# VCISwang/STCD

Hardware: AMD Instinct MI355X
Metric: image-pairs/sec (256x256 bf16 SiamUnet_diff train) (higher is better)
Workload: dtype bf16; 1 GPU; SiamUnet_diff(3,2) 256x256 full training step (fwd + cross_entropy + bwd + AdamW), 16 pairs/GPU, synthetic LEVIR-CD-shaped pairs resident in HBM; global_batch=16, image=256, parallelism=dp1

## Files before the change

stcd_amd/csrc/common.h:

```cpp
#pragma once
#include <hip/hip_runtime.h>
#include <stdint.h>
#include <stdio.h>
#include <stdlib.h>
#include <string>
#include <string.h>

#include "../../include/stcd_hip.h"

namespace stcd {

typedef __bf16 bf16;

enum DType { F32 = STCD_DTYPE_F32, BF16 = STCD_DTYPE_BF16 };
inline size_t dsize(int dt) { return dt == BF16 ? 2 : 4; }

void set_error(const std::string& msg);

static inline int env_int(const char* name, int dflt) { const char* v = getenv(name); return v ? atoi(v) : dflt; }
static inline bool env_flag(const char* name, bool dflt) { const char* v = getenv(name); return v && v[0] == (dflt ? '0' : '1') ? !dflt : dflt; }

#define STCD_CHECK_AS(fn, cond, msg)                                       \
    do {                                                                   \
        if (!(cond)) {                                                     \
// ... 336 lines not shown
};
ConvDmaPlan conv_dma_plan(const stcd_conv_geom& g, const ConvMfmaPlan& p);
int launch_conv_dma(const stcd_conv_geom& g, const ConvMfmaPlan& p, const ConvDmaPlan& dp, const ConvArgs& c);

bool conv_small_ok(const stcd_conv_geom& g, const ConvMfmaPlan& p);
int conv_small_blocks(const stcd_conv_geom& g, int groups);
int launch_conv_small(const stcd_conv_geom& g, const ConvArgs& c);
bool conv_small_call_ok(const stcd_conv_geom& g, int groups, const XfSrc* xf);
bool conv_small_bwdsum_ok(const stcd_conv_geom& g);
struct WgradMfmaPlan {
    int WCI = 1, NTW = 1, gx = 1, gy = 1, gz = 1;
    int64_t slab_floats = 0;
    int wi_valid = 0;
    int gemm = 0;
    int dma = 0;
    bool ok = false;
};
WgradMfmaPlan wgrad_mfma_plan(const stcd_conv_geom& g, int kpad, int wld, bool allow_wide = false, int force_co64 = -1);
int launch_wgrad_mfma(const stcd_conv_geom& g, const WgradMfmaPlan& p, const void* in, const void* dout, float* slab,
                      int kpad, int wld, hipStream_t s);
struct WgradJob {
    stcd_conv_geom g;
    int64_t in_off, dout_off, slab_off;
    int kpad, wld;
    int dymin, dxmin, HH, HWp;
    int tiles_x, tiles_y, ntiles;
    int xrow_bytes;
    int x_bytes, y_bytes;
    int co_valid;
    unsigned in_bytes, dout_bytes;
    int gx, gy, gz;
    int start;
    int lds_bytes;
    int wi_valid;
    int dma_L, dma_nk;
    int pad_;
    int64_t xf_stat_off, xf_mask_off;
    int xf_C, xf_groups, xf_npg, pad2_;
};
WgradMfmaPlan wgrad_gemm_plan(const stcd_conv_geom& g, int kpad, int wld);
WgradMfmaPlan wgrad_dma_plan(const stcd_conv_geom& g, int kpad, int wld);
void wgrad_dma_set_split(WgradMfmaPlan& p, const stcd_conv_geom& g, int S, int kpad, int wld);
WgradJob wgrad_dma_make_job(const stcd_conv_geom& g, const WgradMfmaPlan& p, int64_t in_off, int64_t dout_off, int64_t slab_off,
                            int kpad, int wld);
int launch_wgrad_dma_group(const WgradJob* jobs_dev, int njobs, int total_blocks, const char* base, hipStream_t s);
struct WgradKernel {
    enum Kind { TILE, GEMM, DMA } kind = TILE;
    int WCI = 0, NTW = 0; bool t9 = false, xf = false;
    int W = 0;
    bool operator==(const WgradKernel& o) const { return kind == o.kind && WCI == o.WCI && NTW == o.NTW && t9 == o.t9 && xf == o.xf && W == o.W; }
};
struct WgradXf { int64_t stat_off = -1, mask_off = -1; int C = 0, groups = 1, npg = 1; };
WgradKernel wgrad_kernel_of(const WgradMfmaPlan& p, const stcd_conv_geom& g, bool xf);
bool wgrad_kernel_takes_xf(const WgradKernel& k);
void wgrad_kernel_name(const WgradKernel& k, bool grouped, char out[64]);
int wgrad_variant_slots(const WgradKernel& k, int lds_bytes);
WgradJob wgrad_job(const WgradKernel& k, const stcd_conv_geom& g, const WgradMfmaPlan& p, int64_t in_off, int64_t dout_off,
                   int64_t slab_off, int kpad, int wld, const WgradXf* xf = nullptr);
int launch_wgrad_jobs(const WgradKernel& k, const WgradJob* jobs_dev, int njobs, int total_blocks, int lds_bytes, const char* base,
                      hipStream_t s);
struct PackSpec;
struct ReduceJob {
// ... 293 lines not shown
```

stcd_amd/csrc/engine.hip:

```cpp
#include <algorithm>
#include <climits>
#include <cstdint>
#include <array>
#include <cstring>
#include <memory>
#include <vector>

#include "common.h"

namespace stcd {

static thread_local std::string g_err;
void set_error(const std::string& msg) { g_err = msg; }

enum ConvKind { K_CONV3 = 0, K_CONVT3_S1 = 1, K_UPCONV = 2, K_CONV1 = 3, K_CONVT2 = 4, K_CONV3_S2 = 5, K_CONV1_S2 = 6, K_STEM7 = 7 };

struct TRef { int64_t off = -1; int ld = 0; };
struct GRef { int64_t off = -1; int ld = 0; int64_t goff = 0; };

static inline int round8(int c) { return (c + 7) & ~7; }

struct ConvW {
    std::string name;
    int kind = 0, cin = 0, cout = 0;
// ... 232 lines not shown
    int64_t jobs_total[2] = {0, 0}, jobs_off[2] = {-1, -1};
    const void* jobs_uploaded_ws = nullptr;
    uint64_t weights_tag = 0, packed_tag = 0;
    const void* packed_ws = nullptr; const void* packed_params = nullptr; int packed_level = -1;
    TRef X0, G, finalIn, dFinalIn;
    int Hs[5] = {0}, Ws[5] = {0};
    TRef D[4], dD[4], P[4], dP[4];
    int64_t zero_begin = -1, zero_end = -1;
    int64_t final_bias_acc = -1;
    std::vector<BiasJob> bias_jobs; int64_t bias_jobs_off = -1;
    int64_t masks = -1, dwe_begin = -1, dwe_end = -1, scratch8 = -1;
    int use_mfma = 1, use_small = 1, use_wgroup = 1, use_res = 1, use_skip_fused = 1, use_act_fuse = 1, use_gemm = 1, use_skip_recompute = 1, use_bwdsum = 1, use_bwdsum_res = 0, use_tile = 1, use_halo = 0;
    int wg_side_on = 1;
    static constexpr int WG_SIDE_DIV = 4;
    static constexpr int WGROUP_ROUNDS = 1, WGROUP_MIN_TILES = 8;
    hipStream_t wg_side = nullptr; hipEvent_t wg_fork = nullptr, wg_join = nullptr; int wg_side_dev = -1;
};

}

using namespace stcd;
struct stcd_engine : stcd_engine_impl {};

namespace stcd {

static const int ENC_STAGE_CONVS[4] = {2, 2, 3, 3};
static const int ENC_C[4] = {16, 32, 64, 128};
static const int SKIP_IDX[4] = {1, 3, 6, 9};

static void add_param(stcd_engine& e, const std::string& name, std::initializer_list<int64_t> shape, int64_t* off_out) {
// ... 417 lines not shown
static void split_tile_group(const stcd_engine& e, int stage, const WgradGroup& G, const std::vector<WgradOp*>& ops) {
    int64_t W = 0;
    for (const WgradOp* op : ops) W += wgrad_ntiles(op->g) * op->plan.gy * op->plan.gz;
    int slots = wgrad_variant_slots(G.kernel, G.lds_bytes);
    if (stage == 0 && e.wg_side_on && fc_family(e)) slots = std::max(64, slots / stcd_engine_impl::WG_SIDE_DIV);
    const int64_t rounds = stcd_engine_impl::WGROUP_ROUNDS;
    const int64_t tpb = std::max<int64_t>(stcd_engine_impl::WGROUP_MIN_TILES, (W + rounds * slots - 1) / (rounds * slots));
    for (WgradOp* op : ops) {
        const int64_t slab = wgrad_slab_floats(e, *op);
        int64_t gx = std::max<int64_t>(1, (wgrad_ntiles(op->g) + tpb - 1) / tpb);
        gx = std::min<int64_t>(gx, std::max<int64_t>(1, ((int64_t)32 << 20) / (slab * 4)));
        op->plan.gx = (int)gx;
        op->plan.slab_floats = gx * slab;
    }
}
static void choose_wgroup_splits(stcd_engine& e) {
    for (int st = 0; st < 2; ++st)
        for (size_t gi = 0; gi < e.wgroups[st].size(); ++gi) {
            WgradGroup& G = e.wgroups[st][gi];
            std::vector<WgradOp*> ops;
            for (WgradOp* op : e.wgrad_ops)
                if (op->stage == st && op->group == (int)gi) ops.push_back(op);
            for (const WgradOp* op : ops)
                G.lds_bytes = std::max(G.lds_bytes, wgrad_job_of(e, G.kernel, *op, 0, 0, 0).lds_bytes);
            if (G.kernel.kind == WgradKernel::DMA) split_dma_group(e, ops);
            else if (G.kernel.kind == WgradKernel::TILE) split_tile_group(e, st, G, ops);
        }
}

static void take_wgrad_slabs(stcd_engine& e, Planner& ws) {
    for (WgradOp* op : e.wgrad_ops) {
        if (!op->plan.ok) continue;
        op->slab = ws.take(op->plan.slab_floats * 4);
        if (op->group < 0) continue;
        WgradGroup& G = e.wgroups[op->stage][op->group];
        WgradJob j = wgrad_job_of(e, G.kernel, *op, op->in_off, op->dout_off, op->slab);
        j.start = G.total_blocks;
        G.total_blocks += j.gx * j.gy * j.gz;
        G.jobs.push_back(j);
        double fl, by;
        conv_work(e, op->g, op->kreal, op->nreal, &fl, &by);
        G.flops += fl; G.bytes += by;
// ... 45 lines not shown
        const int k = op->group == last->group ? 1 : 0;
        tot[k] = append_reduce_job(part[k], tot[k], e.rjobs[1][part[0].size() + part[1].size()]);
    }
    if (part[0].empty() || part[1].empty()) return;
    e.rjobs[1] = part[0];
    e.rjobs[1].insert(e.rjobs[1].end(), part[1].begin(), part[1].end());
    e.rj_split = (int)part[0].size(); e.wg_final_group = last->group;
    e.rj_total_early = tot[0]; e.rj_total_final = tot[1];
}

static void build_wgrad_jobs(stcd_engine& e, Planner& ws) {
    for (int st = 0; st < 2; ++st) { e.rjobs[st].clear(); e.rjobs_total[st] = 0; e.wgroups[st].clear(); }
    e.rj_split = 0; e.wg_final_group = -1; e.rj_total_early = e.rj_total_final = 0;
    if (e.dt == BF16 && e.use_mfma) {
        if (e.use_wgroup) { form_wgroups(e); choose_wgroup_splits(e); }
        take_wgrad_slabs(e, ws);
        build_reduce_tables(e);
        split_reduce_final(e);
        for (int st = 0; st < 2; ++st) {
            e.rjobs_off[st] = ws.take((int64_t)e.rjobs[st].size() * sizeof(ReduceJob) + 16);
            for (WgradGroup& G : e.wgroups[st]) G.table_off = ws.take((int64_t)G.jobs.size() * sizeof(WgradJob) + 16);
        }
    }
    for (int st = 0; st < 2; ++st) e.wrun.groups[st].assign(e.wgroups[st].size(), WgradRun::Group());
}

static void build_filter_pack_jobs(stcd_engine& e, Planner& ws) {
    for (int with_dgrad = 0; with_dgrad < 2; ++with_dgrad) {
        std::vector<PackJob>& jobs = e.jobs[with_dgrad];
        jobs.clear();
// ... 38 lines not shown
                }
                push(j);
            }
        }
        e.jobs_total[with_dgrad] = cur;
        e.jobs_off[with_dgrad] = ws.take((int64_t)jobs.size() * sizeof(PackJob) + 16);
    }
}

static int configure_fcsiam(stcd_engine& e, int B, int H, int W) {
    const int64_t T = (int64_t)dsize(e.dt);
    const int ND = fc_dates(e);
    e.Hs[0] = H; e.Ws[0] = W;
    for (int s = 0; s < 4; ++s) { e.Hs[s + 1] = e.Hs[s] / 2; e.Ws[s + 1] = e.Ws[s] / 2; }
    Planner ws(e);
    auto add_drop = [&](const std::string& name, int rows, int C) {
        DropP d; d.name = name; d.rows = rows; d.C = C; d.off = e.drop_floats;
        e.drop_floats += (int64_t)rows * C;
        e.drops.push_back(d);
        return (int)e.drops.size() - 1;
    };

    e.X0 = ws.plain(ND * B, H, W, 8);
    for (int s = 0; s < 4; ++s) {
        int Cd = ENC_C[s] + (e.arch == STCD_ARCH_CONC ? 2 : 1) * ENC_C[s];
        e.D[s] = ws.plain(B, e.Hs[s], e.Ws[s], Cd);
        e.dD[s] = ws.plain(B, e.Hs[s], e.Ws[s], Cd);
        e.P[s] = ws.plain(ND * B, e.Hs[s + 1], e.Ws[s + 1], ENC_C[s]);
        e.dP[s] = ws.plain(ND * B, e.Hs[s + 1], e.Ws[s + 1], ENC_C[s]);
    }
// ... 2028 lines not shown
        else {
            launch_slice(dt, c.at(st.ddst.off), st.ddst.ld, c.at(e.g_pool_idc.off), e.g_pool_idc.ld, (int64_t)st.N * (st.h / 2) * (st.w / 2), st.C, 1, s);
            launch_maxpool3_bwd(dt, c.at<unsigned char>(e.g_pool_idx), c.at(st.ddst.off), st.ddst.ld, c.at(st.dsrc.off), st.dsrc.ld, st.N, st.h, st.w, st.C, s);
        }
    }
    if (stage_tail(c, 0, nullptr, false, finish_biases)) return 1;
    STCD_HIP(hipGetLastError());
    return 0;
}

#include "engine_cf.inl"

static void reset_plan(stcd_engine& e) {
    e.enc.clear(); e.dec.clear(); e.ups.clear();
    e.drops.clear(); e.drop_floats = 0;
    e.conv_ops.clear(); e.wgrad_ops.clear(); e.slab_floats = 0; e.wg_last_op = nullptr;
    e.ws_tensors.clear(); e.bias_jobs.clear();
    e.g_fwd.clear(); e.sn_order.clear();
    if (e.cf) cf_reset_plan(*e.cf);
}

}

extern "C" {

const char* stcd_last_error(void) { return stcd::g_err.c_str(); }
int stcd_abi_version(void) { return STCD_ABI_VERSION; }

static void engine_env_switches(stcd_engine* e) {
    e->use_mfma = !env_flag("STCD_FORCE_REF_KERNELS", false);
    e->use_small = !env_flag("STCD_NO_SMALL_KERNEL", false);
// ... 460 lines not shown
    STCD_CHECK((g->hm - 1) * g->out_stride + g->oy0 < g->ho && (g->wm - 1) * g->out_stride + g->ox0 < g->wo,
               "output positions exceed the output buffer");
    return 0;
}
static int op_dma_splits(const stcd_conv_geom& g, const WgradMfmaPlan& p) {
    const int64_t M = (int64_t)g.n * g.hi * g.wi;
    return (int)std::max<int64_t>(1, std::min<int64_t>(256 / std::max(1, p.gy * p.gz), M / 512));
}
int64_t stcd_op_scratch_bytes(const stcd_conv_geom* g) {
    if (!g) return 0;
    ConvMfmaPlan p = conv_mfma_plan(*g);
    WgradMfmaPlan w = wgrad_mfma_plan(*g, g->ci, g->co), ww = wgrad_mfma_plan(*g, g->ci, g->co, true);
    WgradMfmaPlan wg = wgrad_gemm_plan(*g, g->ci, g->co);
    WgradMfmaPlan wd = wgrad_dma_plan(*g, g->ci, g->co);
    if (wd.ok) wgrad_dma_set_split(wd, *g, op_dma_splits(*g, wd), g->ci, g->co);
    return std::max<int64_t>(p.wf_elems * 2, std::max(std::max(std::max(w.slab_floats, ww.slab_floats), wg.ok ? wg.slab_floats : 0), wd.ok ? wd.slab_floats : 0) * 4) + 1024;
}
int stcd_op_conv(int dtype, int impl, const stcd_conv_geom* g, const void* in, const float* w, const float* bias,
                 void* out, void* scratch, int64_t scratch_bytes, void* hip_stream) {
    if (check_geom(g)) return 1;
    STCD_CHECK(in && w && out, "null pointer argument");
    if (impl == 1 || impl == 2 || impl == 3 || impl == 6 || impl == 8) {
        STCD_CHECK(dtype == STCD_DTYPE_BF16, "the MFMA implementation is bf16 only");
        ConvOp op;
        op.g = *g;
        op.plan = conv_mfma_plan(*g);
        const ConvMfmaPlan& p = op.plan;
        STCD_CHECK(p.ok, "geometry not supported by the MFMA kernel");
        STCD_CHECK(scratch && scratch_bytes >= p.wf_elems * 2, "scratch too small for the fragment-order filter");
        launch_pack_frag(*g, p, w, g->ci, g->co, scratch, (hipStream_t)hip_stream);
        ConvArgs a;
// ... 112 lines not shown
}
int stcd_op_wgrad(int dtype, int impl, const stcd_conv_geom* g, const void* in, const void* dout, float* dw, void* scratch,
                  int64_t scratch_bytes, void* hip_stream) {
    if (check_geom(g)) return 1;
    STCD_CHECK(in && dout && dw, "null pointer argument");
    if (impl == 1 || impl == 4 || impl == 5) {
        STCD_CHECK(dtype == STCD_DTYPE_BF16, "the MFMA implementation is bf16 only");
        WgradMfmaPlan p = wgrad_mfma_plan(*g, g->ci, g->co, impl >= 4, impl == 5 ? 1 : 0);
        STCD_CHECK(p.ok, "geometry not supported by the MFMA kernel");
        STCD_CHECK(scratch && scratch_bytes >= p.slab_floats * 4, "scratch too small for the partial slabs");
        STCD_CHECK(launch_wgrad_mfma(*g, p, in, dout, (float*)scratch, g->ci, g->co, (hipStream_t)hip_stream) == 0, "LDS budget exceeded");
        launch_reduce_dw((const float*)scratch, p.gx, *g, g->ci, g->co, g->ci, g->co, nullptr, dw, (hipStream_t)hip_stream);
        STCD_HIP(hipGetLastError());
        return 0;
    }
    if (impl == 3 || impl == 7) {
        STCD_CHECK(dtype == STCD_DTYPE_BF16, "the MFMA implementation is bf16 only");
        WgradMfmaPlan p = impl == 7 ? wgrad_dma_plan(*g, g->ci, g->co) : wgrad_gemm_plan(*g, g->ci, g->co);
        STCD_CHECK(p.ok, impl == 7 ? "geometry not supported by the LDS-DMA weight-gradient kernel (stride 1, full map >= 64 wide, Ci % 256 == 0, Co % 256 == 0)"
                                   : "geometry not supported by the GEMM weight-gradient kernel (one tap, Ci >= 64, Co >= 64)");
        if (impl == 7) wgrad_dma_set_split(p, *g, op_dma_splits(*g, p), g->ci, g->co);
        const int64_t table = (p.slab_floats * 4 + 255) & ~(int64_t)255;
        STCD_CHECK(scratch && scratch_bytes >= table + (int64_t)sizeof(WgradJob), "scratch too small for the partial slabs + job table");
        const WgradKernel k = wgrad_kernel_of(p, *g, false);
        const WgradJob j = wgrad_job(k, *g, p, (int64_t)(intptr_t)in, (int64_t)(intptr_t)dout, (int64_t)(intptr_t)scratch, g->ci, g->co);
        STCD_HIP(hipMemcpyAsync((char*)scratch + table, &j, sizeof(j), hipMemcpyHostToDevice, (hipStream_t)hip_stream));
        STCD_HIP(hipStreamSynchronize((hipStream_t)hip_stream));
        STCD_CHECK(launch_wgrad_jobs(k, (const WgradJob*)((char*)scratch + table), 1, p.gx * p.gy * p.gz, j.lds_bytes, nullptr, (hipStream_t)hip_stream) == 0, "LDS budget exceeded");
        launch_reduce_dw((const float*)scratch, p.gx, *g, g->ci, g->co, g->ci, g->co, nullptr, dw, (hipStream_t)hip_stream);
        STCD_HIP(hipGetLastError());
        return 0;
    }
    STCD_CHECK(impl == 0, "impl must be 0 (reference FMA), 1 / 4 (MFMA tile kernel, 4: wide tile allowed), 3 (MFMA position-GEMM kernel) or 7 (LDS-DMA kernel)");
    STCD_HIP(hipMemsetAsync(dw, 0, (size_t)g->ntaps * g->ci * g->co * 4, (hipStream_t)hip_stream));
    launch_wgrad_ref(dtype, *g, in, dout, dw, g->ci, g->co, (hipStream_t)hip_stream);
    STCD_HIP(hipGetLastError());
    return 0;
}

}
```

stcd_amd/csrc/kernels_conv_mfma.hip:

```cpp
#include "common.h"

namespace stcd {

typedef __attribute__((ext_vector_type(8))) __bf16 bf16x8;
typedef __attribute__((ext_vector_type(4))) float f32x4;
typedef __attribute__((ext_vector_type(4))) unsigned u32x4;

struct ConvMfmaArgs {
    stcd_conv_geom g;
    const bf16* in;
    const bf16* wf;
    const float* bias;
    void* out;
    int out_nchw;
    int CiB, nchunks, KS;
    int modeB;
    int NTtot;
    int dymin, dxmin, HH, HWp, swmask;
    int tiles_x, tiles_y;
    int halo_bytes, wbuf_bytes;
    int tap[9];
};

static inline void fill_taps(const stcd_conv_geom& g, int* tap) {
// ... 858 lines not shown
    a.xf_stat_off = -1; a.xf_mask_off = -1; a.xf_C = 0; a.xf_groups = 1; a.xf_npg = 1; a.pad2_ = 0;
    return a;
}

#define WG_DISPATCH(W_, N_, T_, WHAT)                                       \
    do {                                                                    \
        if ((W_) == 4 && (N_) == 4) { if (T_) { WHAT(4, 4, true); } else { WHAT(4, 4, false); } }   \
        else if ((W_) == 4) { if (T_) { WHAT(4, 2, true); } else { WHAT(4, 2, false); } }           \
        else if ((W_) == 1 && (N_) == 1) { if (T_) { WHAT(1, 1, true); } else { WHAT(1, 1, false); } }   \
        else if ((W_) == 1) { if (T_) { WHAT(1, 2, true); } else { WHAT(1, 2, false); } }           \
        else if ((N_) == 1) { if (T_) { WHAT(2, 1, true); } else { WHAT(2, 1, false); } }           \
        else { if (T_) { WHAT(2, 2, true); } else { WHAT(2, 2, false); } }                          \
    } while (0)

int wgrad_variant_slots(const WgradKernel& k, int lds_bytes) {
    int dev = 0, cus = 256, per_cu = 2;
    if (hipGetDevice(&dev) != hipSuccess) { (void)hipGetLastError(); return 512; }
    hipDeviceProp_t prop;
    if (hipGetDeviceProperties(&prop, dev) == hipSuccess) cus = prop.multiProcessorCount;
#define WG_OCC(W_, N_, T_) \
    if (hipOccupancyMaxActiveBlocksPerMultiprocessor(&per_cu, k_wgrad_group<W_, N_, T_>, 256, (size_t)lds_bytes) != hipSuccess) per_cu = 2
    WG_DISPATCH(k.WCI, k.NTW, k.t9, WG_OCC);
#undef WG_OCC
    (void)hipGetLastError();
    return std::max(1, per_cu) * cus;
}

#define WG_LDS_ATTR(K_)                                                                                                                  \
    do {                                                                                                                                 \
        static bool attr_set = false;                                                                                                    \
// ... 1412 lines not shown
    const size_t lds = (size_t)2 * 2 * (T / 32) * (64 * 64 + 8 * 32);
    if (W == 4) {
        static bool attr_set = false;
        if (!attr_set) { (void)hipFuncSetAttribute((const void*)k_wgrad_gemm<4>, hipFuncAttributeMaxDynamicSharedMemorySize, 160 * 1024); attr_set = true; }
        k_wgrad_gemm<4><<<(unsigned)total_blocks, 256, lds, s>>>(jobs_dev, njobs, base);
    } else {
        k_wgrad_gemm<2><<<(unsigned)total_blocks, 256, lds, s>>>(jobs_dev, njobs, base);
    }
    return 0;
}

WgradKernel wgrad_kernel_of(const WgradMfmaPlan& p, const stcd_conv_geom& g, bool xf) {
    WgradKernel k;
    if (p.dma) k.kind = WgradKernel::DMA;
    else if (p.gemm) { k.kind = WgradKernel::GEMM; k.W = p.gemm; }
    else { k.WCI = p.WCI; k.NTW = p.NTW; k.t9 = g.ntaps == 9; k.xf = xf; }
    return k;
}
bool wgrad_kernel_takes_xf(const WgradKernel& k) { return k.kind == WgradKernel::TILE && k.WCI < 4 && k.NTW < 4; }
void wgrad_kernel_name(const WgradKernel& k, bool grouped, char out[64]) {
    if (k.kind == WgradKernel::DMA) snprintf(out, 64, "k_wgrad_dma");
    else if (k.kind == WgradKernel::GEMM) snprintf(out, 64, "k_wgrad_gemm<%d>", k.W);
    else if (grouped) snprintf(out, 64, "k_wgrad_group<%d, %d, %s>", k.WCI, k.NTW, k.t9 ? "true" : "false");
    else snprintf(out, 64, "k_wgrad_mfma<%d, %d>", k.WCI, k.NTW);
}
WgradJob wgrad_job(const WgradKernel& k, const stcd_conv_geom& g, const WgradMfmaPlan& p, int64_t in_off, int64_t dout_off,
                   int64_t slab_off, int kpad, int wld, const WgradXf* xf) {
    if (k.kind == WgradKernel::DMA) return wgrad_dma_make_job(g, p, in_off, dout_off, slab_off, kpad, wld);
    if (k.kind == WgradKernel::GEMM) return wgrad_gemm_make_job(g, p, in_off, dout_off, slab_off, kpad, wld);
    WgradJob a = wgrad_make_job(g, p, in_off, dout_off, slab_off, kpad, wld);
    if (k.xf && xf) {
        a.xf_stat_off = xf->stat_off; a.xf_mask_off = xf->mask_off; a.xf_C = xf->C; a.xf_groups = xf->groups; a.xf_npg = xf->npg;
        a.lds_bytes = std::max(a.lds_bytes, 2 * (a.x_bytes + a.y_bytes) + xf->groups * 2 * xf->C * 4);
    }
    return a;
}
int launch_wgrad_jobs(const WgradKernel& k, const WgradJob* jobs_dev, int njobs, int total_blocks, int lds_bytes, const char* base,
                      hipStream_t s) {
    if (k.kind == WgradKernel::DMA) return launch_wgrad_dma_group(jobs_dev, njobs, total_blocks, base, s);
    if (k.kind == WgradKernel::GEMM) return launch_wgrad_gemm_group(k.W, jobs_dev, njobs, total_blocks, base, s);
    return launch_wgrad_group(k.WCI, k.NTW, k.t9, jobs_dev, njobs, total_blocks, lds_bytes, base, s, k.xf);
}

}
```

Baseline: 8022 image-pairs/sec.

## Add LDS-DMA ring-buffered weight-gradient kernel for small-channel 3x3 convs

Adds a new weight-gradient kernel for 3x3 stride-1 convolutions with at most 32 input and output channels. It streams input and output-gradient tiles into a multi-deep LDS ring through buffer-load DMA, reads them with transposed LDS reads, and accumulates with MFMA. It then reduces across waves in LDS and writes per-block partial slabs. The planner moves eligible tile-kernel wgrad ops onto this kernel when the grid is large enough and re-forms the wgrad groups. The aim is to hide load latency for the high-resolution, low-channel layers, at the cost of a new kernel path with a bank-conflict-sensitive layout and different split heuristics.

```diff
diff --git a/stcd_amd/csrc/common.h b/stcd_amd/csrc/common.h
--- a/stcd_amd/csrc/common.h
+++ b/stcd_amd/csrc/common.h
@@ -374,6 +374,7 @@
     int wi_valid = 0;
     int gemm = 0;
     int dma = 0;
+    int ring = 0;
     bool ok = false;
 };
 WgradMfmaPlan wgrad_mfma_plan(const stcd_conv_geom& g, int kpad, int wld, bool allow_wide = false, int force_co64 = -1);
@@ -404,8 +405,15 @@
 WgradJob wgrad_dma_make_job(const stcd_conv_geom& g, const WgradMfmaPlan& p, int64_t in_off, int64_t dout_off, int64_t slab_off,
                             int kpad, int wld);
 int launch_wgrad_dma_group(const WgradJob* jobs_dev, int njobs, int total_blocks, const char* base, hipStream_t s);
+WgradMfmaPlan wgrad_ring_plan(const stcd_conv_geom& g, int kpad, int wld);
+int wgrad_ring_slots(int WCI, int NTW);
+int wgrad_ring_gx(const WgradMfmaPlan& p, int64_t ntiles, int slots);
+WgradJob wgrad_ring_make_job(const stcd_conv_geom& g, const WgradMfmaPlan& p, int64_t in_off, int64_t dout_off, int64_t slab_off,
+                             int kpad, int wld);
+void launch_wgrad_ring_put_job(const WgradJob& j, WgradJob* dst, hipStream_t s);
+int launch_wgrad_ring_group(int WCI, int NTW, const WgradJob* jobs_dev, int njobs, int total_blocks, const char* base, hipStream_t s);
 struct WgradKernel {
-    enum Kind { TILE, GEMM, DMA } kind = TILE;
+    enum Kind { TILE, GEMM, DMA, RING } kind = TILE;
     int WCI = 0, NTW = 0; bool t9 = false, xf = false;
     int W = 0;
     bool operator==(const WgradKernel& o) const { return kind == o.kind && WCI == o.WCI && NTW == o.NTW && t9 == o.t9 && xf == o.xf && W == o.W; }
diff --git a/stcd_amd/csrc/engine.hip b/stcd_amd/csrc/engine.hip
--- a/stcd_amd/csrc/engine.hip
+++ b/stcd_amd/csrc/engine.hip
@@ -270,6 +270,8 @@
     int wg_side_on = 1;
     static constexpr int WG_SIDE_DIV = 4;
     static constexpr int WGROUP_ROUNDS = 1, WGROUP_MIN_TILES = 8;
+    bool wg_ring = false;
+    static constexpr int WG_RING_CLASSES = 0xF, WG_RING_MIN_BLOCKS = 256;
     hipStream_t wg_side = nullptr; hipEvent_t wg_fork = nullptr, wg_join = nullptr; int wg_side_dev = -1;
 };
 
@@ -717,7 +719,18 @@
         op->plan.slab_floats = gx * slab;
     }
 }
-static void choose_wgroup_splits(stcd_engine& e) {
+static void split_ring_group(const stcd_engine& e, int stage, const WgradGroup& G, const std::vector<WgradOp*>& ops) {
+    int64_t W = 0;
+    for (const WgradOp* op : ops) W += wgrad_ntiles(op->g);
+    int slots = wgrad_variant_slots(G.kernel, G.lds_bytes);
+    if (stage == 0 && e.wg_side_on && fc_family(e)) slots = std::max(64, slots / stcd_engine_impl::WG_SIDE_DIV);
+    for (WgradOp* op : ops) {
+        const int64_t nt = wgrad_ntiles(op->g);
+        const int share = (int)std::max<int64_t>(1, slots * nt / std::max<int64_t>(1, W));
+        op->plan.gx = std::min(op->plan.gx, wgrad_ring_gx(op->plan, nt, share));
+    }
+}
+static void choose_wgroup_splits(stcd_engine& e, bool ring_only = false) {
     for (int st = 0; st < 2; ++st)
         for (size_t gi = 0; gi < e.wgroups[st].size(); ++gi) {
             WgradGroup& G = e.wgroups[st][gi];
@@ -726,9 +739,25 @@
                 if (op->stage == st && op->group == (int)gi) ops.push_back(op);
             for (const WgradOp* op : ops)
                 G.lds_bytes = std::max(G.lds_bytes, wgrad_job_of(e, G.kernel, *op, 0, 0, 0).lds_bytes);
-            if (G.kernel.kind == WgradKernel::DMA) split_dma_group(e, ops);
+            if (G.kernel.kind == WgradKernel::RING) { if (ring_only) split_ring_group(e, st, G, ops); }
+            else if (ring_only) continue;
+            else if (G.kernel.kind == WgradKernel::DMA) split_dma_group(e, ops);
             else if (G.kernel.kind == WgradKernel::TILE) split_tile_group(e, st, G, ops);
         }
+}
+static bool move_to_ring(stcd_engine& e) {
+    bool any = false;
+    for (WgradOp* op : e.wgrad_ops) {
+        if (!op->plan.ok || op->group < 0 || op->xf.C > 0) continue;
+        if (wgrad_kernel_of(op->plan, op->g, false).kind != WgradKernel::TILE) continue;
+        const PackSpec& f = e.convs[op->conv].fwd;
+        const WgradMfmaPlan r = wgrad_ring_plan(op->g, f.kpad, f.wld);
+        if (!r.ok || !((stcd_engine_impl::WG_RING_CLASSES >> (2 * (op->g.ci > 16) + (op->g.co > 16))) & 1)) continue;
+        if (!(e.debug_flags & 8) && wgrad_ring_gx(r, wgrad_ntiles(op->g), 1 << 30) < stcd_engine_impl::WG_RING_MIN_BLOCKS) continue;
+        op->plan.ring = 1; op->plan.WCI = r.WCI; op->plan.NTW = r.NTW; op->plan.gy = op->plan.gz = 1;
+        any = true;
+    }
+    return any;
 }
 
 static void take_wgrad_slabs(stcd_engine& e, Planner& ws) {
@@ -804,6 +833,11 @@
     e.rj_split = 0; e.wg_final_group = -1; e.rj_total_early = e.rj_total_final = 0;
     if (e.dt == BF16 && e.use_mfma) {
         if (e.use_wgroup) { form_wgroups(e); choose_wgroup_splits(e); }
+        if (e.use_wgroup && e.wg_ring && !(e.debug_flags & 4) && move_to_ring(e)) {
+            for (int st = 0; st < 2; ++st) e.wgroups[st].clear();
+            form_wgroups(e);
+            choose_wgroup_splits(e, true);
+        }
         take_wgrad_slabs(e, ws);
         build_reduce_tables(e);
         split_reduce_final(e);
@@ -872,6 +906,7 @@
     e.Hs[0] = H; e.Ws[0] = W;
     for (int s = 0; s < 4; ++s) { e.Hs[s + 1] = e.Hs[s] / 2; e.Ws[s + 1] = e.Ws[s] / 2; }
     Planner ws(e);
+    e.wg_ring = true;
     auto add_drop = [&](const std::string& name, int rows, int C) {
         DropP d; d.name = name; d.rows = rows; d.C = C; d.off = e.drop_floats;
         e.drop_floats += (int64_t)rows * C;
@@ -2930,7 +2965,7 @@
 static void reset_plan(stcd_engine& e) {
     e.enc.clear(); e.dec.clear(); e.ups.clear();
     e.drops.clear(); e.drop_floats = 0;
-    e.conv_ops.clear(); e.wgrad_ops.clear(); e.slab_floats = 0; e.wg_last_op = nullptr;
+    e.conv_ops.clear(); e.wgrad_ops.clear(); e.slab_floats = 0; e.wg_last_op = nullptr; e.wg_ring = false;
     e.ws_tensors.clear(); e.bias_jobs.clear();
     e.g_fwd.clear(); e.sn_order.clear();
     if (e.cf) cf_reset_plan(*e.cf);
@@ -3421,7 +3456,9 @@
     WgradMfmaPlan wg = wgrad_gemm_plan(*g, g->ci, g->co);
     WgradMfmaPlan wd = wgrad_dma_plan(*g, g->ci, g->co);
     if (wd.ok) wgrad_dma_set_split(wd, *g, op_dma_splits(*g, wd), g->ci, g->co);
-    return std::max<int64_t>(p.wf_elems * 2, std::max(std::max(std::max(w.slab_floats, ww.slab_floats), wg.ok ? wg.slab_floats : 0), wd.ok ? wd.slab_floats : 0) * 4) + 1024;
+    WgradMfmaPlan wr = wgrad_ring_plan(*g, g->ci, g->co);
+    const int64_t slabs = std::max(std::max(std::max(std::max(w.slab_floats, ww.slab_floats), wg.ok ? wg.slab_floats : 0), wd.ok ? wd.slab_floats : 0), wr.ok ? wr.slab_floats : 0);
+    return std::max<int64_t>(p.wf_elems * 2, slabs * 4) + 1024;
 }
 int stcd_op_conv(int dtype, int impl, const stcd_conv_geom* g, const void* in, const float* w, const float* bias,
                  void* out, void* scratch, int64_t scratch_bytes, void* hip_stream) {
@@ -3564,6 +3601,20 @@
         STCD_HIP(hipGetLastError());
         return 0;
     }
+    if (impl == 9) {
+        STCD_CHECK(dtype == STCD_DTYPE_BF16, "the MFMA implementation is bf16 only");
+        const WgradMfmaPlan p = wgrad_ring_plan(*g, g->ci, g->co);
+        STCD_CHECK(p.ok, "geometry not supported by the LDS-DMA ring weight-gradient kernel (3x3 stride 1 from the map's origin, Ci <= 32, Co <= 32)");
+        const int64_t table = (p.slab_floats * 4 + 255) & ~(int64_t)255;
+        STCD_CHECK(scratch && scratch_bytes >= table + (int64_t)sizeof(WgradJob), "scratch too small for the partial slabs + job table");
+        const WgradKernel k = wgrad_kernel_of(p, *g, false);
+        const WgradJob j = wgrad_job(k, *g, p, (int64_t)(intptr_t)in, (int64_t)(intptr_t)dout, (int64_t)(intptr_t)scratch, g->ci, g->co);
+        launch_wgrad_ring_put_job(j, (WgradJob*)((char*)scratch + table), (hipStream_t)hip_stream);
+        STCD_CHECK(launch_wgrad_jobs(k, (const WgradJob*)((char*)scratch + table), 1, p.gx, j.lds_bytes, nullptr, (hipStream_t)hip_stream) == 0, "launch refused");
+        launch_reduce_dw((const float*)scratch, p.gx, *g, g->ci, g->co, g->ci, g->co, nullptr, dw, (hipStream_t)hip_stream);
+        STCD_HIP(hipGetLastError());
+        return 0;
+    }
     if (impl == 3 || impl == 7) {
         STCD_CHECK(dtype == STCD_DTYPE_BF16, "the MFMA implementation is bf16 only");
         WgradMfmaPlan p = impl == 7 ? wgrad_dma_plan(*g, g->ci, g->co) : wgrad_gemm_plan(*g, g->ci, g->co);
@@ -3581,7 +3632,7 @@
         STCD_HIP(hipGetLastError());
         return 0;
     }
-    STCD_CHECK(impl == 0, "impl must be 0 (reference FMA), 1 / 4 (MFMA tile kernel, 4: wide tile allowed), 3 (MFMA position-GEMM kernel) or 7 (LDS-DMA kernel)");
+    STCD_CHECK(impl == 0, "impl must be 0 (reference FMA), 1 / 4 (MFMA tile kernel, 4: wide tile allowed), 3 (MFMA position-GEMM kernel) 7 (LDS-DMA kernel) or 9 (LDS-DMA ring kernel)");
     STCD_HIP(hipMemsetAsync(dw, 0, (size_t)g->ntaps * g->ci * g->co * 4, (hipStream_t)hip_stream));
     launch_wgrad_ref(dtype, *g, in, dout, dw, g->ci, g->co, (hipStream_t)hip_stream);
     STCD_HIP(hipGetLastError());
diff --git a/stcd_amd/csrc/kernels_conv_mfma.hip b/stcd_amd/csrc/kernels_conv_mfma.hip
--- a/stcd_amd/csrc/kernels_conv_mfma.hip
+++ b/stcd_amd/csrc/kernels_conv_mfma.hip
@@ -896,6 +896,7 @@
     } while (0)
 
 int wgrad_variant_slots(const WgradKernel& k, int lds_bytes) {
+    if (k.kind == WgradKernel::RING) return wgrad_ring_slots(k.WCI, k.NTW);
     int dev = 0, cus = 256, per_cu = 2;
     if (hipGetDevice(&dev) != hipSuccess) { (void)hipGetLastError(); return 512; }
     hipDeviceProp_t prop;
@@ -2338,6 +2339,7 @@
     WgradKernel k;
     if (p.dma) k.kind = WgradKernel::DMA;
     else if (p.gemm) { k.kind = WgradKernel::GEMM; k.W = p.gemm; }
+    else if (p.ring) { k.kind = WgradKernel::RING; k.WCI = p.WCI; k.NTW = p.NTW; k.t9 = true; }
     else { k.WCI = p.WCI; k.NTW = p.NTW; k.t9 = g.ntaps == 9; k.xf = xf; }
     return k;
 }
@@ -2345,6 +2347,7 @@
 void wgrad_kernel_name(const WgradKernel& k, bool grouped, char out[64]) {
     if (k.kind == WgradKernel::DMA) snprintf(out, 64, "k_wgrad_dma");
     else if (k.kind == WgradKernel::GEMM) snprintf(out, 64, "k_wgrad_gemm<%d>", k.W);
+    else if (k.kind == WgradKernel::RING) snprintf(out, 64, "k_wgrad_ring<%d, %d>", k.WCI, k.NTW);
     else if (grouped) snprintf(out, 64, "k_wgrad_group<%d, %d, %s>", k.WCI, k.NTW, k.t9 ? "true" : "false");
     else snprintf(out, 64, "k_wgrad_mfma<%d, %d>", k.WCI, k.NTW);
 }
@@ -2352,6 +2355,7 @@
                    int64_t slab_off, int kpad, int wld, const WgradXf* xf) {
     if (k.kind == WgradKernel::DMA) return wgrad_dma_make_job(g, p, in_off, dout_off, slab_off, kpad, wld);
     if (k.kind == WgradKernel::GEMM) return wgrad_gemm_make_job(g, p, in_off, dout_off, slab_off, kpad, wld);
+    if (k.kind == WgradKernel::RING) return wgrad_ring_make_job(g, p, in_off, dout_off, slab_off, kpad, wld);
     WgradJob a = wgrad_make_job(g, p, in_off, dout_off, slab_off, kpad, wld);
     if (k.xf && xf) {
         a.xf_stat_off = xf->stat_off; a.xf_mask_off = xf->mask_off; a.xf_C = xf->C; a.xf_groups = xf->groups; a.xf_npg = xf->npg;
@@ -2363,6 +2367,7 @@
                       hipStream_t s) {
     if (k.kind == WgradKernel::DMA) return launch_wgrad_dma_group(jobs_dev, njobs, total_blocks, base, s);
     if (k.kind == WgradKernel::GEMM) return launch_wgrad_gemm_group(k.W, jobs_dev, njobs, total_blocks, base, s);
+    if (k.kind == WgradKernel::RING) return launch_wgrad_ring_group(k.WCI, k.NTW, jobs_dev, njobs, total_blocks, base, s);
     return launch_wgrad_group(k.WCI, k.NTW, k.t9, jobs_dev, njobs, total_blocks, lds_bytes, base, s, k.xf);
 }
 
diff --git a/stcd_amd/csrc/kernels_wgrad_ring.hip b/stcd_amd/csrc/kernels_wgrad_ring.hip
--- /dev/null
+++ b/stcd_amd/csrc/kernels_wgrad_ring.hip
@@ -0,0 +1,352 @@
+#include <algorithm>
+#include <cstring>
+
+#include "common.h"
+
+namespace stcd {
+
+typedef __attribute__((ext_vector_type(8))) __bf16 bf16x8;
+typedef __attribute__((ext_vector_type(4))) __bf16 bf16x4;
+typedef __attribute__((ext_vector_type(4))) float f32x4;
+
+constexpr int RG_XROW = 768, RG_XSUB = 8192;
+constexpr int RG_YROW = 512, RG_YSUB = 4096;
+#define RG_LDS(P_) ((__attribute__((address_space(3))) void*)(P_))
+
+constexpr int rg_pix(int p) { return (p >> 4) * 512 + ((p >> 2) & 1) * 256 + ((p & 3) + 4 * ((p >> 3) & 1)) * 32; }
+constexpr int rg_inv(int o) { return (o >> 9) * 16 + ((o >> 7) & 1) * 8 + ((o >> 8) & 1) * 4 + ((o >> 5) & 3); }
+constexpr bool rg_half_ok(int a, int row, int pitch) {
+    unsigned long long used = 0;
+    for (int l = 0; l < 32; ++l) {
+        const int addr = row * pitch + rg_pix(a + 8 * (l >> 4) + ((l & 15) >> 2)) + 8 * (l & 3);
+        for (int w = 0; w < 2; ++w) {
+            const int b = (addr / 4 + w) % 64;
+            if ((used >> b) & 1) return false;
+            used |= 1ull << b;
+        }
+    }
+    return true;
+}
+constexpr bool rg_layout_ok() {
+    for (int p = 0; p < 18; ++p)
+        if (rg_inv(rg_pix(p)) != p || rg_pix(p) + 32 > RG_XROW) return false;
+    for (int p = 0; p < 16; ++p)
+        if (rg_pix(p) + 32 > RG_YROW) return false;
+    for (int half = 0; half < 2; ++half)
+        for (int rd = 0; rd < 2; ++rd) {
+            for (int tdx = 0; tdx < 3; ++tdx)
+                if (!rg_half_ok(tdx + 4 * rd, half, RG_XROW)) return false;
+            if (!rg_half_ok(4 * rd, half, RG_YROW)) return false;
+        }
+    return true;
+}
+static_assert(RG_XROW % 256 == 0 && RG_YROW % 256 == 0 && RG_XSUB % 1024 == 0 && RG_YSUB % 1024 == 0 && 10 * RG_XROW <= RG_XSUB &&
+              8 * RG_YROW <= RG_YSUB, "ring image: rows keep their bank phase, sub-images are whole DMA instructions");
+static_assert(rg_layout_ok(), "ring image: a 32-lane half of a transposed read must touch every LDS bank exactly once");
+
+template <int WCI, int NTW>
+struct RingCfg {
+    static constexpr int D = (WCI == 2 && NTW == 2) ? 3 : 4;
+    static constexpr int BLOCKS = (WCI == 1 && NTW == 1) ? 3 : 2;
+    static constexpr int NX = 2 * WCI, NY = NTW, NI = NX + NY;
+    static constexpr int XB = WCI * RG_XSUB, YB = NTW * RG_YSUB, BUF = XB + YB;
+    static constexpr int WK = 4 / WCI;
+    static constexpr int RED = (WK - 1) * WCI * 9 * NTW * 4 * 64 * 4;
+    static constexpr int LDS = D * BUF > RED ? D * BUF : RED;
+    static_assert(BLOCKS * LDS <= 160 * 1024, "ring: blocks per CU x LDS");
+};
+
+template <int OFF>
+__device__ __forceinline__ bf16x8 rg_tr(unsigned a0, unsigned a1) {
+    bf16x4 lo, hi;
+    asm volatile("ds_read_b64_tr_b16 %0, %2 offset:%4\n\tds_read_b64_tr_b16 %1, %3 offset:%4"
+                 : "=&v"(lo), "=&v"(hi) : "v"(a0), "v"(a1), "n"(OFF) : "memory");
+    bf16x8 f;
+    f[0] = lo[0]; f[1] = lo[1]; f[2] = lo[2]; f[3] = lo[3];
+    f[4] = hi[0]; f[5] = hi[1]; f[6] = hi[2]; f[7] = hi[3];
+    return f;
+}
+#define RG_LGKM(N_)                                                   \
+    do {                                                              \
+        asm volatile("s_waitcnt lgkmcnt(%0)" ::"n"(N_) : "memory");   \
+        __builtin_amdgcn_sched_barrier(0);                            \
+    } while (0)
+
+template <int WCI, int NTW>
+__device__ __forceinline__ void ring_body(const WgradJob& a, const char* base, const int bx) {
+    using C = RingCfg<WCI, NTW>;
+    constexpr int D = C::D, NX = C::NX, NI = C::NI, WK = C::WK;
+    extern __shared__ __attribute__((aligned(16))) char smem[];
+    const int tid = threadIdx.x, lane = tid & 63;
+    const int wid = __builtin_amdgcn_readfirstlane(tid >> 6);
+    const int wci = wid % WCI, wk = wid / WCI;
+    const int grp = lane >> 4, li = lane & 15, qrow = li >> 2, pcol = li & 3;
+    const int g_hi = a.g.hi, g_wi = a.g.wi, g_ho = a.g.ho, g_wo = a.g.wo, g_hm = a.g.hm, g_wm = a.g.wm, ldi = a.g.ldi, ldo = a.g.ldo;
+    const int wi_valid = a.wi_valid, tiles_x = a.tiles_x, tiles_y = a.tiles_y, ntiles = a.ntiles, step = a.gx;
+
+    int voff[NI], vyx[NI];
+#pragma unroll
+    for (int i = 0; i < NI; ++i) {
+        if (i < NX) {
+            const int k = i * 4 + wid, L = (k & 7) * 1024 + lane * 16;
+            const int row = L / RG_XROW, o = L - row * RG_XROW, p = rg_inv(o & ~31), ch = (k >> 3) * 16 + ((o >> 4) & 1) * 8;
+            const bool ok = row < 10 && p < 18 && ch < a.g.ci;
+            vyx[i] = ok ? (((row - 1) << 16) | ((p - 1) & 0xffff)) : (0x4000 << 16);
+            voff[i] = ((row * g_wi + p) * ldi + ch) * 2;
+        } else {
+            const int k = (i - NX) * 4 + wid, L = (k & 3) * 1024 + lane * 16;
+            const int row = L / RG_YROW, o = L - row * RG_YROW, p = rg_inv(o & ~31), ch = (k >> 2) * 16 + ((o >> 4) & 1) * 8;
+            const bool ok = ch < a.co_valid;
+            vyx[i] = ok ? ((row << 16) | p) : (0x4000 << 16);
+            voff[i] = ((row * g_wo + p) * ldo + ch) * 2;
+        }
+    }
+    const int64_t lead = ((int64_t)g_wi + 1) * ldi * 2;
+    const __amdgpu_buffer_rsrc_t xrs = __builtin_amdgcn_make_buffer_rsrc(
+        const_cast<char*>(base + a.in_off) - lead, (short)0, (int)(a.in_bytes + (unsigned)lead), 0x00020000);
+    const __amdgpu_buffer_rsrc_t yrs = __builtin_amdgcn_make_buffer_rsrc(
+        const_cast<char*>(base + a.dout_off), (short)0, (int)a.dout_bytes, 0x00020000);
+
+    const int tiles_img = tiles_x * tiles_y;
+    const int dn = step / tiles_img, drem = step - dn * tiles_img, dty = drem / tiles_x, dtx = drem - dty * tiles_x;
+    int rt = bx, rn = rt / tiles_img;
+    int ry, rx;
+    { const int trem = rt - rn * tiles_img; ry = trem / tiles_x; rx = trem - ry * tiles_x; }
+#define RG_REQ(BUF_)                                                                                                   \
+    do {                                                                                                               \
+        const bool live_ = rt < ntiles;                                                                                \
+        const int my0_ = ry * 8, mx0_ = rx * 16;                                                                       \
+        const int xs_ = __builtin_amdgcn_readfirstlane(                                                                \
+            live_ ? (int)(unsigned)(((((int64_t)rn * g_hi + my0_) * g_wi + mx0_) * ldi) * 2) : 0);                     \
+        const int ys_ = __builtin_amdgcn_readfirstlane(                                                                \
+            live_ ? (int)(unsigned)(((((int64_t)rn * g_ho + my0_) * g_wo + mx0_) * ldo) * 2) : 0);                     \
+        char* const dst_ = smem + (BUF_) * C::BUF;                                                                     \
+        _Pragma("unroll") for (int i = 0; i < NI; ++i) {                                                               \
+            const int y_ = my0_ + (vyx[i] >> 16), x_ = mx0_ + (int)(short)(vyx[i] & 0xffff);                           \
+            if (i < NX) {                                                                                              \
+                const bool ok_ = live_ && (unsigned)y_ < (unsigned)g_hi && (unsigned)x_ < (unsigned)wi_valid;          \
+                __builtin_amdgcn_raw_ptr_buffer_load_lds(xrs, RG_LDS(dst_ + (i * 4 + wid) * 1024), 16,                 \
+                                                         ok_ ? voff[i] : (int)0x80000000u, xs_, 0, 0);                 \
+            } else {                                                                                                   \
+                const bool ok_ = live_ && (unsigned)y_ < (unsigned)g_hm && (unsigned)x_ < (unsigned)g_wm;              \
+                __builtin_amdgcn_raw_ptr_buffer_load_lds(yrs, RG_LDS(dst_ + C::XB + ((i - NX) * 4 + wid) * 1024), 16,  \
+                                                         ok_ ? voff[i] : (int)0x80000000u, ys_, 0, 0);                 \
+            }                                                                                                          \
+        }                                                                                                              \
+        rt += step;                                                                                                    \
+        rx += dtx; if (rx >= tiles_x) { rx -= tiles_x; ++ry; }                                                         \
+        ry += dty; if (ry >= tiles_y) { ry -= tiles_y; ++rn; }                                                         \
+        rn += dn;                                                                                                      \
+    } while (0)
+
+    const int frow = grp >> 1, fx0 = 8 * (grp & 1) + qrow;
+    const unsigned lds0 = (unsigned)(uintptr_t)(__attribute__((address_space(3))) char*)smem;
+    unsigned xo0[3], xo1[3];
+#pragma unroll
+    for (int dx = 0; dx < 3; ++dx) {
+        xo0[dx] = lds0 + (unsigned)(wci * RG_XSUB + frow * RG_XROW + rg_pix(fx0 + dx) + 8 * pcol);
+        xo1[dx] = lds0 + (unsigned)(wci * RG_XSUB + frow * RG_XROW + rg_pix(fx0 + dx + 4) + 8 * pcol);
+    }
+    const unsigned yo0 = lds0 + (unsigned)(frow * RG_YROW + rg_pix(fx0) + 8 * pcol), yo1 = lds0 + (unsigned)(frow * RG_YROW + rg_pix(fx0 + 4) + 8 * pcol);
+
+    f32x4 acc[9][NTW];
+#pragma unroll
+    for (int t = 0; t < 9; ++t)
+#pragma unroll
+        for (int n_ = 0; n_ < NTW; ++n_) acc[t][n_] = f32x4{0.f, 0.f, 0.f, 0.f};
+
+#define RG_KSTEP(KS_)                                                                                                  \
+    do {                                                                                                               \
+        bf16x8 bfr[NTW], afr[9];                                                                                       \
+        _Pragma("unroll") for (int n_ = 0; n_ < NTW; ++n_) {                                                           \
+            if (n_ == 0) bfr[n_] = rg_tr<C::XB + (KS_) * 2 * RG_YROW>(yo0 + yb, yo1 + yb);                              \
+            else bfr[n_] = rg_tr<C::XB + RG_YSUB + (KS_) * 2 * RG_YROW>(yo0 + yb, yo1 + yb);                            \
+        }                                                                                                              \
+        _Pragma("unroll") for (int dx = 0; dx < 3; ++dx) afr[dx] = rg_tr<((KS_) * 2 + 0) * RG_XROW>(xo0[dx] + xb, xo1[dx] + xb);     \
+        _Pragma("unroll") for (int dx = 0; dx < 3; ++dx) afr[3 + dx] = rg_tr<((KS_) * 2 + 1) * RG_XROW>(xo0[dx] + xb, xo1[dx] + xb); \
+        _Pragma("unroll") for (int dx = 0; dx < 3; ++dx) afr[6 + dx] = rg_tr<((KS_) * 2 + 2) * RG_XROW>(xo0[dx] + xb, xo1[dx] + xb); \
+        _Pragma("unroll") for (int r_ = 0; r_ < 3; ++r_) {                                                             \
+            if (r_ == 0) RG_LGKM(12); else if (r_ == 1) RG_LGKM(6); else RG_LGKM(0);                                   \
+            _Pragma("unroll") for (int dx = 0; dx < 3; ++dx)                                                           \
+                _Pragma("unroll") for (int n_ = 0; n_ < NTW; ++n_)                                                     \
+                    acc[r_ * 3 + dx][n_] = __builtin_amdgcn_mfma_f32_16x16x32_bf16(afr[r_ * 3 + dx], bfr[n_], acc[r_ * 3 + dx][n_], 0, 0, 0); \
+        }                                                                                                              \
+        __builtin_amdgcn_sched_barrier(0);                                                                             \
+    } while (0)
+
+#pragma unroll
+    for (int k = 0; k < D; ++k) RG_REQ(k);
+    int buf = 0;
+    for (int tile = bx; tile < ntiles; tile += step) {
+        asm volatile("s_waitcnt vmcnt(%0)" ::"n"(NI * (D - 1)) : "memory");
+        __builtin_amdgcn_sched_barrier(0);
+        __builtin_amdgcn_s_barrier();
+        __builtin_amdgcn_sched_barrier(0);
+        const unsigned xb = (unsigned)(buf * C::BUF + wk * 2 * RG_XROW), yb = (unsigned)(buf * C::BUF + wk * 2 * RG_YROW);
+        RG_KSTEP(0);
+        if constexpr (WK == 2) RG_KSTEP(2);
+        barrier_lds();
+        __builtin_amdgcn_sched_barrier(0);
+        RG_REQ(buf);
+        buf = buf + 1 == D ? 0 : buf + 1;
+    }
+    asm volatile("s_waitcnt vmcnt(0)" ::: "memory");
+    __builtin_amdgcn_sched_barrier(0);
+    __syncthreads();
+#undef RG_KSTEP
+#undef RG_REQ
+
+    float* red = reinterpret_cast<float*>(smem);
+    constexpr int PERW = 9 * NTW * 4 * 64;
+    if (wk > 0) {
+        float* dst = red + ((wk - 1) * WCI + wci) * PERW + lane;
+#pragma unroll
+        for (int t = 0; t < 9; ++t)
+#pragma unroll
+            for (int n_ = 0; n_ < NTW; ++n_)
+#pragma unroll
+                for (int j = 0; j < 4; ++j) dst[((t * NTW + n_) * 4 + j) * 64] = acc[t][n_][j];
+    }
+    __syncthreads();
+    if (wk == 0) {
+#pragma unroll 1
+        for (int w = 1; w < WK; ++w) {
+            const float* src = red + ((w - 1) * WCI + wci) * PERW + lane;
+#pragma unroll
+            for (int t = 0; t < 9; ++t)
+#pragma unroll
+                for (int n_ = 0; n_ < NTW; ++n_)
+#pragma unroll
+                    for (int j = 0; j < 4; ++j) acc[t][n_][j] += src[((t * NTW + n_) * 4 + j) * 64];
+        }
+        float* slab = reinterpret_cast<float*>(const_cast<char*>(base) + a.slab_off) + (int64_t)bx * 9 * a.kpad * a.wld;
+#pragma unroll
+        for (int t = 0; t < 9; ++t)
+#pragma unroll
+            for (int n_ = 0; n_ < NTW; ++n_)
+#pragma unroll
+                for (int j = 0; j < 4; ++j) {
+                    const int ci = wci * 16 + 4 * grp + j, co = n_ * 16 + li;
+                    if (ci < a.kpad && co < a.wld) slab[((int64_t)t * a.kpad + ci) * a.wld + co] = acc[t][n_][j];
+                }
+    }
+}
+
+template <int WCI, int NTW>
+__global__ void __launch_bounds__(256, (WCI == 1 && NTW == 1) ? 3 : 2)
+k_wgrad_ring(const WgradJob* __restrict__ jobs, int njobs, const char* base) {
+    static_assert(RingCfg<WCI, NTW>::BLOCKS == ((WCI == 1 && NTW == 1) ? 3 : 2), "launch bounds");
+    int lo = 0, hi = njobs - 1;
+    while (lo < hi) {
+        const int mid = (lo + hi + 1) >> 1;
+        if (jobs[mid].start <= (int)blockIdx.x) lo = mid; else hi = mid - 1;
+    }
+    const WgradJob& a = jobs[lo];
+    ring_body<WCI, NTW>(a, base, blockIdx.x - a.start);
+}
+
+#define RG_DISPATCH(W_, N_, WHAT)                          \
+    do {                                                   \
+        if ((W_) == 1 && (N_) == 1) { WHAT(1, 1); }        \
+        else if ((W_) == 1) { WHAT(1, 2); }                \
+        else if ((N_) == 1) { WHAT(2, 1); }                \
+        else { WHAT(2, 2); }                               \
+    } while (0)
+
+static int ring_depth(int WCI, int NTW) {
+#define RG_D(W_, N_) return RingCfg<W_, N_>::D
+    RG_DISPATCH(WCI, NTW, RG_D);
+#undef RG_D
+}
+static int ring_lds(int WCI, int NTW) {
+#define RG_L(W_, N_) return RingCfg<W_, N_>::LDS
+    RG_DISPATCH(WCI, NTW, RG_L);
+#undef RG_L
+}
+static void ring_lds_attr() {
+    static bool attr_set = false;
+    if (attr_set) return;
+    for (const void* f : {(const void*)k_wgrad_ring<1, 1>, (const void*)k_wgrad_ring<1, 2>, (const void*)k_wgrad_ring<2, 1>, (const void*)k_wgrad_ring<2, 2>})
+        (void)hipFuncSetAttribute(f, hipFuncAttributeMaxDynamicSharedMemorySize, 160 * 1024);
+    attr_set = true;
+}
+
+int wgrad_ring_slots(int WCI, int NTW) {
+    int dev = 0, cus = 256, per_cu = 2;
+    if (hipGetDevice(&dev) != hipSuccess) { (void)hipGetLastError(); return 512; }
+    hipDeviceProp_t prop;
+    if (hipGetDeviceProperties(&prop, dev) == hipSuccess) cus = prop.multiProcessorCount;
+    ring_lds_attr();
+#define RG_OCC(W_, N_)                                                                                                        \
+    do {                                                                                                                      \
+        if (hipOccupancyMaxActiveBlocksPerMultiprocessor(&per_cu, k_wgrad_ring<W_, N_>, 256, (size_t)RingCfg<W_, N_>::LDS) != hipSuccess) per_cu = 2; \
+        per_cu = std::min(per_cu, RingCfg<W_, N_>::BLOCKS);                                                                   \
+    } while (0)
+    RG_DISPATCH(WCI, NTW, RG_OCC);
+#undef RG_OCC
+    (void)hipGetLastError();
+    return std::max(1, per_cu) * cus;
+}
+
+int wgrad_ring_gx(const WgradMfmaPlan& p, int64_t ntiles, int slots) {
+    const int D = ring_depth(p.WCI, p.NTW);
+    int64_t gx = std::min<int64_t>(slots, std::max<int64_t>(1, ntiles / (2 * D)));
+    return (int)std::max<int64_t>(1, std::min<int64_t>(gx, ntiles));
+}
+
+WgradMfmaPlan wgrad_ring_plan(const stcd_conv_geom& g, int kpad, int wld) {
+    WgradMfmaPlan p;
+    if (g.ntaps != 9 || g.in_stride != 1 || g.out_stride != 1 || g.oy0 != 0 || g.ox0 != 0 || g.hm > g.hi || g.wm > g.wi || g.hm > g.ho || g.wm > g.wo) return p;
+    for (int t = 0; t < 9; ++t)
+        if (g.dy[t] != t / 3 - 1 || g.dx[t] != t % 3 - 1) return p;
+    if (g.hi >= 16384 || g.wi >= 16384 || g.ho >= 16384 || g.wo >= 16384) return p;
+    if (kpad < 1 || wld < 1 || kpad > 32 || wld > 32 || g.ci > 32 || g.co > 32 || g.ci % 8 != 0 || g.ldi % 8 != 0 || g.ldo % 8 != 0) return p;
+    if (((int64_t)g.n * g.hi + 4) * g.wi * g.ldi * 2 >= ((int64_t)1 << 31) || (int64_t)g.n * g.ho * g.wo * g.ldo * 2 >= ((int64_t)1 << 31)) return p;
+    p.ring = 1;
+    p.WCI = g.ci > 16 ? 2 : 1; p.NTW = g.co > 16 ? 2 : 1;
+    p.gy = p.gz = 1;
+    const int64_t ntiles = (int64_t)g.n * ((g.wm + 15) / 16) * ((g.hm + 7) / 8);
+    p.gx = wgrad_ring_gx(p, ntiles, wgrad_ring_slots(p.WCI, p.NTW));
+    p.slab_floats = (int64_t)p.gx * 9 * kpad * wld;
+    p.ok = true;
+    return p;
+}
+
+WgradJob wgrad_ring_make_job(const stcd_conv_geom& g, const WgradMfmaPlan& p, int64_t in_off, int64_t dout_off, int64_t slab_off,
+                             int kpad, int wld) {
+    WgradJob a;
+    memset(&a, 0, sizeof(a));
+    a.g = g;
+    a.in_off = in_off; a.dout_off = dout_off; a.slab_off = slab_off; a.kpad = kpad; a.wld = wld;
+    a.dymin = a.dxmin = -1; a.HH = 10; a.HWp = 18;
+    a.tiles_x = (g.wm + 15) / 16;
+    a.tiles_y = (g.hm + 7) / 8;
+    a.ntiles = g.n * a.tiles_x * a.tiles_y;
+    a.xrow_bytes = RG_XROW;
+    a.x_bytes = p.WCI * RG_XSUB; a.y_bytes = p.NTW * RG_YSUB;
+    a.co_valid = (g.co + 7) & ~7;
+    a.in_bytes = (unsigned)((int64_t)g.n * g.hi * g.wi * g.ldi * 2);
+    a.dout_bytes = (unsigned)((int64_t)g.n * g.ho * g.wo * g.ldo * 2);
+    a.gx = p.gx; a.gy = 1; a.gz = 1; a.start = 0;
+    a.wi_valid = p.wi_valid > 0 ? p.wi_valid : g.wi;
+    a.lds_bytes = ring_lds(p.WCI, p.NTW);
+    a.xf_stat_off = -1; a.xf_mask_off = -1;
+    return a;
+}
+
+__global__ void k_wgrad_ring_put_job(const WgradJob j, WgradJob* dst) {
+    if (threadIdx.x == 0) *dst = j;
+}
+void launch_wgrad_ring_put_job(const WgradJob& j, WgradJob* dst, hipStream_t s) { k_wgrad_ring_put_job<<<1, 64, 0, s>>>(j, dst); }
+
+int launch_wgrad_ring_group(int WCI, int NTW, const WgradJob* jobs_dev, int njobs, int total_blocks, const char* base, hipStream_t s) {
+    if (njobs <= 0 || total_blocks <= 0) return 0;
+    if (WCI < 1 || WCI > 2 || NTW < 1 || NTW > 2) return 1;
+    ring_lds_attr();
+#define RG_GO(W_, N_) k_wgrad_ring<W_, N_><<<(unsigned)total_blocks, 256, (size_t)RingCfg<W_, N_>::LDS, s>>>(jobs_dev, njobs, base)
+    RG_DISPATCH(WCI, NTW, RG_GO);
+#undef RG_GO
+    return 0;
+}
+
+}
```

After: 8080 image-pairs/sec (median of 6 runs). No clear change (+0.7%).
